# bastienjossen/DDL25Spring

Measured on AMD Instinct MI355X. Metric: FedAvg rounds/sec + local samples/sec, ResNet-18 CIFAR-10-shape, 8 clients, higher is better.
Workload: dtype fp32; 1 GPU; model=resnet18-cifar10, global_batch=800, parallelism=fedavg-8clients-dp1, clients=8, local_batch=100, local_epochs=1, samples_per_client=6250, client_slots_per_gpu=8, hip_graphs=True, fp32_conv_math=auto

## Files before the change

### csrc/include/conv_f32_core.h

```cpp
#pragma once
#include "ddl_common.h"

struct ConvF32Args {
  const float* x;
  const float* w;
  const float* dy;
  float* out;
  float* stats;
  const float* bias;
  const float* residual;
  const float* mask;
  const float* in_scale;
  const float* in_shift;
  const float* bn_x;
  const float* bn_mean;
  const float* bn_rstd;
  const float* mask_scale;
  const float* mask_shift;
  float* partial;
  long long partial_cap;
  long long x_gs, w_gs, dy_gs, out_gs, bias_gs, res_gs;
  int G, N, H, W, C, K, R, S, P, Q, stride, pad;
  int relu, accumulate, split_k, res_sub, in_relu;
  int slots;
  float gscale;
  const void* wsplit;
  long long ws_gs;
  const float* dyb_x;
  const float* dyb_coef;
  float* dyb_out;
  int* tickets;
  long long tickets_cap;
};

enum { F_FWD = 0, F_DGRAD = 1, F_WGRAD = 2 };

struct FDiv {
  uint32_t m;
  int s;
};
__host__ __device__ inline FDiv mk_fdiv(uint32_t d) {
  FDiv f;
  if (d <= 1) { f.m = 0; f.s = 0; return f; }
  int l = 0;
  while ((1u << l) < d) ++l;
  f.m = (uint32_t)((((1ull << 32) * ((1ull << l) - d)) / d) + 1);
  f.s = l;
  return f;
}
__device__ __forceinline__ int fdv(int x, FDiv f) {
  if (f.s == 0) return x;
  const uint32_t t = __umulhi((uint32_t)x, f.m);
  return (int)((t + (((uint32_t)x - t) >> 1)) >> (f.s - 1));
}

struct FGeo {
  int Pd, Qd, Kr, nph, phase, split, nsplit, g, p0, q0, tq;
  int pa, pb, Hs, Ws, r0, s0, Rn, Sn;
};

template <int MODE, int BP, int BQ>
__device__ __forceinline__ FGeo fgeo(const ConvF32Args& a, int bx, int by, int g, int gy) {
  FGeo o;
  o.nph = (MODE == F_DGRAD && a.stride == 2) ? 4 : 1;
  o.phase = by % o.nph;
  o.split = by / o.nph;
  o.nsplit = gy / o.nph;
  o.g = g;
  o.pa = o.pb = o.r0 = o.s0 = 0;
  o.Hs = a.H; o.Ws = a.W; o.Rn = a.R; o.Sn = a.S;
  if (MODE == F_FWD) {
    o.Pd = a.K; o.Qd = a.N * a.P * a.Q; o.Kr = a.R * a.S * a.C;
  } else if (MODE == F_DGRAD) {
    o.Pd = a.C;
    if (o.nph == 4) {
      o.pa = o.phase >> 1; o.pb = o.phase & 1;
      o.Hs = (a.H - o.pa + 1) >> 1; o.Ws = (a.W - o.pb + 1) >> 1;
      o.r0 = (o.pa + a.pad) & 1; o.s0 = (o.pb + a.pad) & 1;
      o.Rn = (a.R - o.r0 + 1) >> 1; o.Sn = (a.S - o.s0 + 1) >> 1;
    }
    o.Qd = a.N * o.Hs * o.Ws;
    o.Kr = o.Rn * o.Sn * a.K;
  } else {
    o.Pd = a.K; o.Qd = a.R * a.S * a.C; o.Kr = a.N * a.P * a.Q;
  }
// ... 224 lines not shown
    float* st = a.stats + ((long long)g * a.slots + slot) * 2 * Pd + o.p0 + tid;
    st[0] = t0;
    st[Pd] = t1;
  }
}

template <int MODE, int BP>
__device__ __forceinline__ void fzero_slot(const ConvF32Args& a, const FGeo& o) {
  if (MODE == F_WGRAD || !a.stats || (MODE == F_DGRAD && !a.bn_x)) return;
  const int tid = threadIdx.x;
  if (tid < BP && o.p0 + tid < o.Pd) {
    const int slot = o.phase * (a.slots / o.nph) + o.tq;
    float* st = a.stats + ((long long)o.g * a.slots + slot) * 2 * o.Pd + o.p0 + tid;
    st[0] = 0.f;
    st[o.Pd] = 0.f;
  }
}

template <int MODE, int BP, int BQ>
__global__ __launch_bounds__(256) void convf32_splitk_epilogue(ConvF32Args a) {
  constexpr int WP = BP / 2, WQ = BQ / 2, TP = WP / 16, TQ = WQ / 16;
  __shared__ float red[2 * BP * 2];
  const int tid = threadIdx.x, lane = tid & 63, wid = tid >> 6, wp = wid >> 1, wq = wid & 1;
  const int nph = (MODE == F_DGRAD && a.stride == 2) ? 4 : 1;
  const FGeo o = fgeo<MODE, BP, BQ>(a, blockIdx.x, blockIdx.y, blockIdx.z, nph * a.split_k);
  if (o.q0 >= o.Qd || o.p0 >= o.Pd) {
    fzero_slot<MODE, BP>(a, o);
    return;
  }
  const long long qmax = (long long)a.slots / nph * BQ;
  const long long slice = (long long)a.G * nph * qmax * o.Pd;
  const float* base = a.partial + ((long long)o.g * nph + o.phase) * qmax * o.Pd;
  f4v acc[TP][TQ];
  bool ok[TP][TQ];
  const float* src[TP][TQ];
#pragma unroll
  for (int ti = 0; ti < TP; ++ti)
#pragma unroll
    for (int tj = 0; tj < TQ; ++tj) {
      const int q = o.q0 + wq * WQ + tj * 16 + (lane & 15);
      const int p = o.p0 + wp * WP + ti * 16 + 4 * (lane >> 4);
      ok[ti][tj] = q < o.Qd && p < o.Pd;
      src[ti][tj] = base + (ok[ti][tj] ? (long long)q * o.Pd + p : 0);
      acc[ti][tj] = (f4v){0.f, 0.f, 0.f, 0.f};
    }
  for (int k = 0; k < a.split_k; ++k) {
    f4v v[TP][TQ];
#pragma unroll
    for (int ti = 0; ti < TP; ++ti)
#pragma unroll
      for (int tj = 0; tj < TQ; ++tj)
        v[ti][tj] = ok[ti][tj] ? *(const f4v*)(src[ti][tj] + k * slice) : (f4v){0.f, 0.f, 0.f, 0.f};
#pragma unroll
    for (int ti = 0; ti < TP; ++ti)
#pragma unroll
      for (int tj = 0; tj < TQ; ++tj) acc[ti][tj] += v[ti][tj];
  }
  fepi<MODE, BP, BQ, Lay16<BP, BQ>>(a, o, acc, red);
}


__device__ __forceinline__ void split3(float4 v, s4v& h, s4v& m, s4v& l) {
  const float x[4] = {v.x, v.y, v.z, v.w};
#pragma unroll
  for (int i = 0; i < 4; ++i) {
    const uint32_t u = __float_as_uint(x[i]);
    const float r1 = x[i] - __uint_as_float(u & 0xFFFF0000u);
    const uint32_t um = __float_as_uint(r1);
    const float r2 = r1 - __uint_as_float(um & 0xFFFF0000u);
    h[i] = (short)(u >> 16);
    m[i] = (short)(um >> 16);
    l[i] = (short)(__float_as_uint(r2) >> 16);
  }
}
__device__ __forceinline__ void split1(float x, uint16_t& h, uint16_t& m, uint16_t& l) {
  const uint32_t u = __float_as_uint(x);
  const float r1 = x - __uint_as_float(u & 0xFFFF0000u);
  const uint32_t um = __float_as_uint(r1);
  const float r2 = r1 - __uint_as_float(um & 0xFFFF0000u);
  h = (uint16_t)(u >> 16);
  m = (uint16_t)(um >> 16);
  l = (uint16_t)(__float_as_uint(r2) >> 16);
}
__device__ __forceinline__ s8v cat44(s4v a, s4v b) {
  return __builtin_shufflevector(a, b, 0, 1, 2, 3, 4, 5, 6, 7);
}
```

### csrc/kernels/conv_f32.hip

```cpp
#include "conv_f32_core.h"
#include <cstdlib>

#ifndef F32_PREFETCH
#define F32_PREFETCH 2
#endif

constexpr int FBK = 16;

__device__ __forceinline__ int fswz(int row) { return (row >> 2) & 2; }
__device__ __forceinline__ int lds_off(int row, int ch) { return row * 16 + ((ch ^ fswz(row)) << 2); }

__device__ __forceinline__ int x6_off(int row, int ch, int half) {
  const int f = row & 2;
  const int g = (row ^ (row >> 2)) & 1;
  return row * 32 + 8 * (ch ^ f) + 4 * (half ^ g);
}

template <int MODE, int BP, int BQ, int X6>
__global__ __launch_bounds__(256, (X6 && BP * BQ <= 64 * 128) ? 3 : 2) void convf32_kernel(ConvF32Args a) {
  constexpr int WP = BP / 2, WQ = BQ / 2, TP = WP / 16, TQ = WQ / 16;
  constexpr int RW = X6 ? 32 : 16;
  constexpr int SP = BP * RW, SQ = BQ * RW;
  constexpr int UPK = BP / 64, UQK = BQ / 64;
  constexpr int KUP = BP / 64, KUQ = BQ / 64;
  __shared__ float4 smem4[(2 * (SP + SQ)) / 4];
  float* smem = (float*)smem4;
  __shared__ float xform[2 * 512];

  const int tid = threadIdx.x, lane = tid & 63, wid = tid >> 6, wp = wid >> 1, wq = wid & 1;
  const int gx = gridDim.x, gy = gridDim.y, gz = gridDim.z;
  const int lin = blockIdx.x + gx * (blockIdx.y + gy * blockIdx.z);
  const int u = xcd_remap(lin, gx * gy * gz);
  const int bx = u % gx, by = (u / gx) % gy, g = u / (gx * gy);
  const FGeo o = fgeo<MODE, BP, BQ>(a, bx, by, g, gy);
  const bool split_store = a.split_k > 1;
  if (o.q0 >= o.Qd || o.p0 >= o.Pd) {
    if (!split_store || (a.tickets && o.split == 0)) fzero_slot<MODE, BP>(a, o);
    return;
  }
  const int nk = (o.Kr + FBK - 1) / FBK;
  const int per = (nk + o.nsplit - 1) / o.nsplit;
  const int kt0 = o.split * per, kt1 = min(nk, kt0 + per);

  const int H = a.H, W = a.W, C = a.C, K = a.K, S = a.S, P = a.P, Q = a.Q, st = a.stride, pd = a.pad;
  const float* X = a.x + (long long)g * a.x_gs;
  const float* Wt = a.w + (long long)g * a.w_gs;
  const float* DY = a.dy + (long long)g * a.dy_gs;
  const bool xf = (MODE != F_DGRAD) && a.in_scale != nullptr;
  if (xf) {
    for (int i = tid; i < C; i += 256) {
      xform[i] = a.in_scale[(long long)g * C + i];
      xform[512 + i] = a.in_shift[(long long)g * C + i];
    }
  }
  const bool xrelu = a.in_relu != 0;

  int pk_row[UPK], pk_ch[UPK];
  int pm_rg = 0, pm_kp = 0;
  if constexpr (MODE == F_FWD) {
#pragma unroll
    for (int i = 0; i < UPK; ++i) {
      const int uu = tid + 256 * i;
      pk_row[i] = uu >> 2;
      pk_ch[i] = uu & 3;
    }
  } else {
    pm_kp = tid % (16 / KUP);
    pm_rg = tid / (16 / KUP);
  }
  int qk_row[UQK], qk_ch[UQK], qk_n[UQK], qk_hb[UQK], qk_wb[UQK];
  int qm_rg = 0, qm_kp = 0, qm_r = 0, qm_s = 0, qm_c = 0;
  bool qm_ok = false;
  float qm_sc[4] = {1.f, 1.f, 1.f, 1.f}, qm_sh[4] = {0.f, 0.f, 0.f, 0.f};
  if constexpr (MODE != F_WGRAD) {
    const FDiv dpq = mk_fdiv((uint32_t)(MODE == F_FWD ? P * Q : o.Hs * o.Ws));
    const FDiv dq = mk_fdiv((uint32_t)(MODE == F_FWD ? Q : o.Ws));
    const int PQ = MODE == F_FWD ? P * Q : o.Hs * o.Ws, QQ = MODE == F_FWD ? Q : o.Ws;
#pragma unroll
    for (int i = 0; i < UQK; ++i) {
      const int uu = tid + 256 * i;
      qk_row[i] = uu >> 2;
      qk_ch[i] = uu & 3;
      const int q = o.q0 + qk_row[i];
      if (q < o.Qd) {
        const int n = fdv(q, dpq), rem = q - n * PQ;
        const int y = fdv(rem, dq), xq = rem - y * QQ;
        qk_n[i] = n;
        if (MODE == F_FWD) {
          qk_hb[i] = y * st - pd;
          qk_wb[i] = xq * st - pd;
        } else {
          qk_hb[i] = (o.nph == 4 ? 2 * y + o.pa : y) + pd;
          qk_wb[i] = (o.nph == 4 ? 2 * xq + o.pb : xq) + pd;
        }
      } else {
        qk_n[i] = -1;
        qk_hb[i] = qk_wb[i] = 0;
      }
    }
  } else {
    qm_kp = tid % (16 / KUQ);
    qm_rg = tid / (16 / KUQ);
    const int q = o.q0 + 4 * qm_rg;
    qm_ok = q < o.Qd;
    if (qm_ok) {
      const int tap = q / C;
      qm_c = q - tap * C;
      qm_r = tap / S;
      qm_s = tap - qm_r * S;
    }
  }
  if (xf) __syncthreads();
  if constexpr (MODE == F_WGRAD) {
    if (xf && qm_ok) {
#pragma unroll
      for (int v = 0; v < 4; ++v) { qm_sc[v] = xform[qm_c + v]; qm_sh[v] = xform[512 + qm_c + v]; }
    }
  }
  const FDiv dpix = mk_fdiv((uint32_t)(P * Q)), dpq1 = mk_fdiv((uint32_t)Q);

  constexpr unsigned OOB = 0xFFFFFFF0u;
  const __amdgpu_buffer_rsrc_t rX = __builtin_amdgcn_make_buffer_rsrc(
      (void*)X, 0, (int)((long long)a.N * H * W * C * 4), 0x00020000);
  const __amdgpu_buffer_rsrc_t rW = __builtin_amdgcn_make_buffer_rsrc(
      (void*)Wt, 0, (int)((long long)K * a.R * S * C * 4), 0x00020000);
  const __amdgpu_buffer_rsrc_t rD = __builtin_amdgcn_make_buffer_rsrc(
      (void*)DY, 0, (int)((long long)a.N * P * Q * K * 4), 0x00020000);
  auto bload = [&](const __amdgpu_buffer_rsrc_t& rs, unsigned off) -> float4 {
    const auto v = __builtin_amdgcn_raw_buffer_load_b128(rs, off, 0, 0);
    return __builtin_bit_cast(float4, v);
  };
  constexpr int PF = F32_PREFETCH;
  float4 rpA[2], rqA[2], rpB[2], rqB[2], rpC[2], rqC[2];
  bool qvA[2] = {false, false}, qvB[2] = {false, false}, qvC[2] = {false, false};
  auto load_step = [&](int kt, float4 (&rp)[2], float4 (&rq)[2], bool (&qv)[2]) {
    const int kk0 = kt * FBK;
    if constexpr (MODE == F_FWD) {
#pragma unroll
      for (int i = 0; i < UPK; ++i) {
        const int p = o.p0 + pk_row[i];
        rp[i] = bload(rW, p < o.Pd ? (unsigned)(p * o.Kr + kk0 + 4 * pk_ch[i]) * 4u : OOB);
      }
    } else if constexpr (MODE == F_DGRAD) {
      const int tap = kk0 / K, k0 = kk0 - tap * K;
      const int ir = tap / o.Sn, is = tap - ir * o.Sn;
      const int r = o.r0 + (st == 2 ? 2 : 1) * ir, s = o.s0 + (st == 2 ? 2 : 1) * is;
      const int c = o.p0 + 4 * pm_rg;
#pragma unroll
      for (int j = 0; j < KUP; ++j) {
        const int k = k0 + pm_kp * KUP + j;
        rp[j] = bload(rW, c < C ? (unsigned)(((k * a.R + r) * S + s) * C + c) * 4u : OOB);
      }
    } else {
      const int kch = o.p0 + 4 * pm_rg;
#pragma unroll
      for (int j = 0; j < KUP; ++j) {
        const int pix = kk0 + pm_kp * KUP + j;
        rp[j] = bload(rD, (pix < o.Kr && kch < K) ? (unsigned)(pix * K + kch) * 4u : OOB);
      }
    }
    if constexpr (MODE == F_FWD) {
      const int tap = kk0 / C, c0 = kk0 - tap * C;
      const int r = tap / S, s = tap - r * S;
#pragma unroll
      for (int i = 0; i < UQK; ++i) {
        const int h = qk_hb[i] + r, w = qk_wb[i] + s;
        const bool ok = qk_n[i] >= 0 && (unsigned)h < (unsigned)H && (unsigned)w < (unsigned)W;
        qv[i] = ok;
        rq[i] = bload(rX, ok ? (unsigned)(((qk_n[i] * H + h) * W + w) * C + c0 + 4 * qk_ch[i]) * 4u : OOB);
      }
    } else if constexpr (MODE == F_DGRAD) {
      const int tap = kk0 / K, k0 = kk0 - tap * K;
      const int ir = tap / o.Sn, is = tap - ir * o.Sn;
      const int r = o.r0 + (st == 2 ? 2 : 1) * ir, s = o.s0 + (st == 2 ? 2 : 1) * is;
#pragma unroll
      for (int i = 0; i < UQK; ++i) {
        int ho = qk_hb[i] - r, wo = qk_wb[i] - s;
        bool hit = true;
        if (st == 2) {
          ho >>= 1;
          wo >>= 1;
        } else if (st > 2) {
          hit = ho >= 0 && wo >= 0 && ho % st == 0 && wo % st == 0;
          ho /= st;
          wo /= st;
        }
        const bool ok = hit && qk_n[i] >= 0 && (unsigned)ho < (unsigned)P && (unsigned)wo < (unsigned)Q;
        rq[i] = bload(rD, ok ? (unsigned)(((qk_n[i] * P + ho) * Q + wo) * K + k0 + 4 * qk_ch[i]) * 4u : OOB);
      }
    } else {
#pragma unroll
      for (int j = 0; j < KUQ; ++j) {
        const int pix = kk0 + qm_kp * KUQ + j;
        const int n = fdv(pix, dpix), rem = pix - n * P * Q;
        const int ho = fdv(rem, dpq1), wo = rem - ho * Q;
        const int h = ho * st - pd + qm_r, w = wo * st - pd + qm_s;
        const bool ok = qm_ok && pix < o.Kr && (unsigned)h < (unsigned)H && (unsigned)w < (unsigned)W;
        qv[j] = ok;
        rq[j] = bload(rX, ok ? (unsigned)(((n * H + h) * W + w) * C + qm_c) * 4u : OOB);
      }
    }
  };
  auto xform4 = [&](float4 v, const float* sc, const float* sh) {
    v.x = v.x * sc[0] + sh[0];
    v.y = v.y * sc[1] + sh[1];
    v.z = v.z * sc[2] + sh[2];
    v.w = v.w * sc[3] + sh[3];
    if (xrelu) { v.x = fmaxf(v.x, 0.f); v.y = fmaxf(v.y, 0.f); v.z = fmaxf(v.z, 0.f); v.w = fmaxf(v.w, 0.f); }
    return v;
  };
  auto store_mn = [&](float* img, int rg, int kp, int KU, const float4* v) {
#pragma unroll
    for (int j4 = 0; j4 < 4; ++j4) {
      const int row = 4 * rg + j4;
      const int kk = kp * KU;
      float* d = img + row * 16 + (((kk >> 2) ^ fswz(row)) << 2) + (kk & 3);
      const float e0 = j4 == 0 ? v[0].x : j4 == 1 ? v[0].y : j4 == 2 ? v[0].z : v[0].w;
      if (KU == 2) {
        const float e1 = j4 == 0 ? v[1].x : j4 == 1 ? v[1].y : j4 == 2 ? v[1].z : v[1].w;
        *(float2*)d = make_float2(e0, e1);
      } else {
        *d = e0;
      }
    }
  };
  auto store_k6 = [&](float* img, int row, int ch, float4 v) {
    s4v h, m, l;
    split3(v, h, m, l);
    *(s8v*)(img + x6_off(row, ch, 0)) = cat44(h, m);
    *(s8v*)(img + x6_off(row, ch, 1)) = cat44(l, h);
  };
  auto store_mn6 = [&](float* img, int rg, int kp, int KU, const float4* v) {
#pragma unroll
    for (int j4 = 0; j4 < 4; ++j4) {
      const int row = 4 * rg + j4;
      const int kk = kp * KU, ch = kk >> 2, pos = kk & 3;
      uint16_t* h0 = (uint16_t*)(img + x6_off(row, ch, 0)) + pos;
      uint16_t* h1 = (uint16_t*)(img + x6_off(row, ch, 1)) + pos;
      const float e0 = j4 == 0 ? v[0].x : j4 == 1 ? v[0].y : j4 == 2 ? v[0].z : v[0].w;
      uint16_t ah, am, al;
      split1(e0, ah, am, al);
      if (KU == 2) {
        const float e1 = j4 == 0 ? v[1].x : j4 == 1 ? v[1].y : j4 == 2 ? v[1].z : v[1].w;
        uint16_t bh, bm, bl;
        split1(e1, bh, bm, bl);
        *(uint32_t*)h0 = (uint32_t)ah | ((uint32_t)bh << 16);
        *(uint32_t*)(h0 + 4) = (uint32_t)am | ((uint32_t)bm << 16);
        *(uint32_t*)h1 = (uint32_t)al | ((uint32_t)bl << 16);
        *(uint32_t*)(h1 + 4) = (uint32_t)ah | ((uint32_t)bh << 16);
      } else {
        h0[0] = ah;
        h0[4] = am;
        h1[0] = al;
        h1[4] = ah;
      }
    }
  };
  auto store_step = [&](int buf, int kt, float4 (&rp)[2], float4 (&rq)[2], const bool (&qv)[2]) {
    float* Ps = smem + buf * (SP + SQ);
    float* Qs = Ps + SP;
    if constexpr (MODE == F_FWD) {
#pragma unroll
      for (int i = 0; i < UPK; ++i) {
        if constexpr (X6) store_k6(Ps, pk_row[i], pk_ch[i], rp[i]);
        else *(float4*)(Ps + lds_off(pk_row[i], pk_ch[i])) = rp[i];
      }
    } else {
      if constexpr (X6) store_mn6(Ps, pm_rg, pm_kp, KUP, rp);
      else store_mn(Ps, pm_rg, pm_kp, KUP, rp);
    }
    if constexpr (MODE == F_FWD) {
      if (xf) {
        const int kk0 = kt * FBK, c0 = kk0 - (kk0 / C) * C;
#pragma unroll
        for (int i = 0; i < UQK; ++i) {
          const int c = c0 + 4 * qk_ch[i];
          if (qv[i]) rq[i] = xform4(rq[i], xform + c, xform + 512 + c);
        }
      }
    } else if constexpr (MODE == F_WGRAD) {
      if (xf) {
#pragma unroll
        for (int j = 0; j < KUQ; ++j)
          if (qv[j]) rq[j] = xform4(rq[j], qm_sc, qm_sh);
      }
    }
    if constexpr (MODE != F_WGRAD) {
#pragma unroll
      for (int i = 0; i < UQK; ++i) {
        if constexpr (X6) store_k6(Qs, qk_row[i], qk_ch[i], rq[i]);
        else *(float4*)(Qs + lds_off(qk_row[i], qk_ch[i])) = rq[i];
      }
    } else {
      if constexpr (X6) store_mn6(Qs, qm_rg, qm_kp, KUQ, rq);
      else store_mn(Qs, qm_rg, qm_kp, KUQ, rq);
    }
  };

  f4v acc[TP][TQ];
#pragma unroll
  for (int i = 0; i < TP; ++i)
#pragma unroll
    for (int j = 0; j < TQ; ++j) acc[i][j] = (f4v){0.f, 0.f, 0.f, 0.f};

  auto step = [&](int kt, float4 (&cp)[2], float4 (&cq)[2], bool (&cv)[2], float4 (&np)[2],
                  float4 (&nq)[2], bool (&nv)[2]) {
    const int cur = (kt - kt0) & 1;
    if (kt + PF < kt1) load_step(kt + PF, np, nq, nv);
    const float* Ps = smem + cur * (SP + SQ);
    const float* Qs = Ps + SP;
    if constexpr (X6) {
      s8v a0[TP], a1[TP], b0[TQ], b1[TQ];
#pragma unroll
      for (int ti = 0; ti < TP; ++ti) {
        const int R = wp * WP + ti * 16 + (lane & 15);
        a0[ti] = *(const s8v*)(Ps + x6_off(R, lane >> 4, 0));
        a1[ti] = *(const s8v*)(Ps + x6_off(R, lane >> 4, 1));
      }
#pragma unroll
      for (int tj = 0; tj < TQ; ++tj) {
        const int R = wq * WQ + tj * 16 + (lane & 15);
        b0[tj] = *(const s8v*)(Qs + x6_off(R, lane >> 4, 0));
        b1[tj] = *(const s8v*)(Qs + x6_off(R, lane >> 4, 1));
      }
#pragma unroll
      for (int ti = 0; ti < TP; ++ti)
#pragma unroll
        for (int tj = 0; tj < TQ; ++tj) {
          f4v c = __builtin_amdgcn_mfma_f32_16x16x32_bf16(a1[ti], b0[tj], (f4v){0.f, 0.f, 0.f, 0.f}, 0, 0, 0);
          c = __builtin_amdgcn_mfma_f32_16x16x32_bf16(a0[ti], b1[tj], c, 0, 0, 0);
          c = __builtin_amdgcn_mfma_f32_16x16x32_bf16(a0[ti], b0[tj], c, 0, 0, 0);
#pragma unroll
          for (int v = 0; v < 4; ++v) acc[ti][tj][v] = acc[ti][tj][v] + c[v];
        }
    } else {
      float4 af[TP], bfr[TQ];
#pragma unroll
      for (int ti = 0; ti < TP; ++ti)
        af[ti] = *(const float4*)(Ps + lds_off(wp * WP + ti * 16 + (lane & 15), lane >> 4));
#pragma unroll
      for (int tj = 0; tj < TQ; ++tj)
        bfr[tj] = *(const float4*)(Qs + lds_off(wq * WQ + tj * 16 + (lane & 15), lane >> 4));
#pragma unroll
      for (int s4 = 0; s4 < 4; ++s4)
#pragma unroll
        for (int ti = 0; ti < TP; ++ti)
#pragma unroll
          for (int tj = 0; tj < TQ; ++tj) {
            const float av = s4 == 0 ? af[ti].x : s4 == 1 ? af[ti].y : s4 == 2 ? af[ti].z : af[ti].w;
            const float bv = s4 == 0 ? bfr[tj].x : s4 == 1 ? bfr[tj].y : s4 == 2 ? bfr[tj].z : bfr[tj].w;
            acc[ti][tj] = __builtin_amdgcn_mfma_f32_16x16x4f32(av, bv, acc[ti][tj], 0, 0, 0);
          }
    }
    if (kt + 1 < kt1) store_step(cur ^ 1, kt + 1, cp, cq, cv);
    __syncthreads();
  };
  if (kt0 < kt1) {
    load_step(kt0, rpA, rqA, qvA);
    if (kt0 + 1 < kt1) load_step(kt0 + 1, rpB, rqB, qvB);
    if constexpr (PF == 3) {
      if (kt0 + 2 < kt1) load_step(kt0 + 2, rpC, rqC, qvC);
    }
    store_step(0, kt0, rpA, rqA, qvA);
    __syncthreads();
    if constexpr (PF == 3) {
      for (int kt = kt0; kt < kt1; kt += 3) {
        step(kt, rpB, rqB, qvB, rpA, rqA, qvA);
        if (kt + 1 < kt1) step(kt + 1, rpC, rqC, qvC, rpB, rqB, qvB);
        if (kt + 2 < kt1) step(kt + 2, rpA, rqA, qvA, rpC, rqC, qvC);
      }
    } else {
      for (int kt = kt0; kt < kt1; kt += 2) {
        step(kt, rpB, rqB, qvB, rpA, rqA, qvA);
        if (kt + 1 < kt1) step(kt + 1, rpA, rqA, qvA, rpB, rqB, qvB);
      }
    }
  }

  if (split_store) {
#pragma unroll
    for (int ti = 0; ti < TP; ++ti)
#pragma unroll
      for (int tj = 0; tj < TQ; ++tj) {
        const int q = o.q0 + wq * WQ + tj * 16 + (lane & 15);
        const int p = o.p0 + wp * WP + ti * 16 + 4 * (lane >> 4);
        if (q >= o.Qd || p >= o.Pd) continue;
        if constexpr (MODE == F_WGRAD) {
          float* d = a.partial + ((long long)o.split * a.G + g) * o.Pd * o.Qd;
#pragma unroll
          for (int v = 0; v < 4; ++v)
            if (p + v < o.Pd) d[(long long)(p + v) * o.Qd + q] = acc[ti][tj][v];
        } else {
          const long long qmax = (long long)a.slots / o.nph * BQ;
          float* d = a.partial + (((long long)o.split * a.G + g) * o.nph + o.phase) * qmax * o.Pd;
          *(float4*)(d + (long long)q * o.Pd + p) = make_float4(acc[ti][tj][0], acc[ti][tj][1],
                                                                acc[ti][tj][2], acc[ti][tj][3]);
        }
      }
    if (a.tickets) {
      __threadfence();
      __syncthreads();
      int* const last = (int*)smem;
      int* const ticket = a.tickets + ((long long)g * o.nph + o.phase) * gx + bx;
      if (tid == 0) *last = atomicAdd(ticket, 1) == o.nsplit - 1;
      __syncthreads();
      if (!*last) return;
      __threadfence();
      if constexpr (MODE != F_WGRAD) {
        const long long qmax = (long long)a.slots / o.nph * BQ;
        const long long slice = (long long)a.G * o.nph * qmax * o.Pd;
        const float* base = a.partial + ((long long)g * o.nph + o.phase) * qmax * o.Pd;
#pragma unroll
        for (int ti = 0; ti < TP; ++ti)
#pragma unroll
          for (int tj = 0; tj < TQ; ++tj) {
            const int q = o.q0 + wq * WQ + tj * 16 + (lane & 15);
            const int p = o.p0 + wp * WP + ti * 16 + 4 * (lane >> 4);
            f4v sm = (f4v){0.f, 0.f, 0.f, 0.f};
            if (q < o.Qd && p < o.Pd) {
              const float* src = base + (long long)q * o.Pd + p;
              for (int k = 0; k < o.nsplit; ++k) {
                const float4 v = *(const float4*)(src + k * slice);
                sm[0] += v.x; sm[1] += v.y; sm[2] += v.z; sm[3] += v.w;
              }
            }
            acc[ti][tj] = sm;
          }
        __syncthreads();
        if (tid == 0) *ticket = 0;
        fepi<MODE, BP, BQ, Lay16<BP, BQ>>(a, o, acc, smem);
        return;
      } else {
        const long long per = (long long)o.Pd * o.Qd;
        const float* src = a.partial + (long long)g * per;
        float* dst = a.out + (long long)g * a.out_gs;
        for (int e = tid; e < BP * (BQ / 4); e += 256) {
          const int p = o.p0 + e / (BQ / 4), q = o.q0 + 4 * (e % (BQ / 4));
          if (p >= o.Pd || q >= o.Qd) continue;
          const long long off = (long long)p * o.Qd + q;
          float4 sum = make_float4(0.f, 0.f, 0.f, 0.f);
          for (int k = 0; k < o.nsplit; ++k) {
            const float4 v = *(const float4*)(src + (long long)k * a.G * per + off);
            sum.x += v.x; sum.y += v.y; sum.z += v.z; sum.w += v.w;
          }
          float4 b = a.accumulate ? *(const float4*)(dst + off) : make_float4(0.f, 0.f, 0.f, 0.f);
          b.x += a.gscale * sum.x; b.y += a.gscale * sum.y; b.z += a.gscale * sum.z; b.w += a.gscale * sum.w;
          *(float4*)(dst + off) = b;
        }
        if (tid == 0) *ticket = 0;
      }
    }
    return;
  }
  fepi<MODE, BP, BQ, Lay16<BP, BQ>>(a, o, acc, smem);
}

template <int V>
__global__ __launch_bounds__(256) void convf32_wgrad_reduce(const float* __restrict__ part, float* out,
                                                            long long out_gs, int G, long long nv,
                                                            int splits, int accumulate, float gscale) {
  typedef float vec __attribute__((ext_vector_type(V)));
  const long long per = nv * V;
  GSTRIDE_LOOP(t, (long long)G * nv) {
    const long long g = t / nv, i = (t - g * nv) * V;
    vec s = (vec)(0.f);
    const float* src = part + g * per + i;
    const long long sstride = (long long)G * per;
    int k = 0;
    for (; k + 8 <= splits; k += 8) {
      vec v[8];
#pragma unroll
      for (int j = 0; j < 8; ++j) v[j] = *(const vec*)(src + (long long)(k + j) * sstride);
#pragma unroll
      for (int j = 0; j < 8; ++j) s += v[j];
    }
    for (; k < splits; ++k) s += *(const vec*)(src + (long long)k * sstride);
    float* d = out + g * out_gs + i;
    vec b = accumulate ? *(const vec*)d : (vec)(0.f);
    b += gscale * s;
    *(vec*)d = b;
  }
}

static void launch_wgrad_reduce(const float* part, float* out, long long out_gs, int G, long long n, int splits,
                                int accumulate, float gscale, hipStream_t s) {
  static const long long v4_min = [] {
    const char* e = getenv("DDL_WGRAD_REDUCE_V4_MIN");
    return e ? atoll(e) : 512LL * 256;
  }();
  if ((long long)G * (n / 4) >= v4_min)
    hipLaunchKernelGGL(convf32_wgrad_reduce<4>, dim3(grid_for((long long)G * (n / 4), 256)), dim3(256), 0, s, part,
                       out, out_gs, G, n / 4, splits, accumulate, gscale);
  else
    hipLaunchKernelGGL(convf32_wgrad_reduce<1>, dim3(grid_for((long long)G * n, 256)), dim3(256), 0, s, part, out,
                       out_gs, G, n, splits, accumulate, gscale);
}

DDL_API int ddl_convf32_wgrad_reduce(const float* part, float* out, long long out_gs, int G, long long n, int splits,
                                     int accumulate, float gscale, hipStream_t s) {
  if (n % 4) return (int)hipErrorInvalidValue;
  launch_wgrad_reduce(part, out, out_gs, G, n, splits, accumulate, gscale, s);
  return (int)hipGetLastError();
}

static void fdims(const ConvF32Args& a, int mode, long long& Pd, long long& Qd, long long& Qmax, long long& Kr,
                  int& nph) {
  nph = (mode == F_DGRAD && a.stride == 2) ? 4 : 1;
  if (mode == F_FWD) { Pd = a.K; Qd = Qmax = (long long)a.N * a.P * a.Q; Kr = (long long)a.R * a.S * a.C; }
  else if (mode == F_DGRAD) {
    Pd = a.C;
    const int Hs = nph == 4 ? (a.H + 1) >> 1 : a.H, Ws = nph == 4 ? (a.W + 1) >> 1 : a.W;
    Qd = Qmax = (long long)a.N * Hs * Ws;
    Kr = (long long)a.R * a.S * a.K;
  } else { Pd = a.K; Qd = Qmax = (long long)a.R * a.S * a.C; Kr = (long long)a.N * a.P * a.Q; }
}

DDL_API long long ddl_convf32_slots(const ConvF32Args* ap, int mode, int cfg) {
  long long Pd, Qd, Qmax, Kr;
  int nph;
  fdims(*ap, mode, Pd, Qd, Qmax, Kr, nph);
  const int bq = ((cfg >> 8) & 0xff) * 16;
  if (bq <= 0) return -1;
  return nph * ((Qmax + bq - 1) / bq);
}

DDL_API long long ddl_convf32_workspace(const ConvF32Args* ap, int mode, int cfg) {
  if (ap->split_k <= 1) return 0;
  long long Pd, Qd, Qmax, Kr;
  int nph;
  fdims(*ap, mode, Pd, Qd, Qmax, Kr, nph);
  const int bq = ((cfg >> 8) & 0xff) * 16;
  if (mode == F_WGRAD) return (long long)ap->split_k * ap->G * Pd * Qd;
  const long long qm = (Qmax + bq - 1) / bq * bq;
  return (long long)ap->split_k * ap->G * nph * qm * Pd;
}

template <int MODE, int BP, int BQ, int X6>
static int launch_tile(ConvF32Args a, hipStream_t s) {
  long long Pd, Qd, Qmax, Kr;
  int nph;
  fdims(a, MODE, Pd, Qd, Qmax, Kr, nph);
  const long long ntp = (Pd + BP - 1) / BP, ntq = (Qmax + BQ - 1) / BQ;
  a.slots = (int)(nph * ntq);
  const int split = a.split_k < 1 ? 1 : a.split_k;
  a.split_k = split;
  if (split > 1) {
    const long long need = MODE == F_WGRAD ? (long long)split * a.G * Pd * Qd
                                           : (long long)split * a.G * nph * ntq * BQ * Pd;
    if (!a.partial || need > a.partial_cap) return (int)hipErrorInvalidValue;
  }
  const dim3 grid((unsigned)(ntp * ntq), (unsigned)(nph * split), (unsigned)a.G);
  if (split == 1 || (long long)a.G * nph * ntp * ntq > a.tickets_cap) a.tickets = nullptr;
  hipLaunchKernelGGL((convf32_kernel<MODE, BP, BQ, X6>), grid, dim3(256), 0, s, a);
  hipError_t e = hipGetLastError();
  if (e != hipSuccess || split == 1 || a.tickets) return (int)e;
  if (MODE == F_WGRAD) {
    launch_wgrad_reduce((const float*)a.partial, a.out, a.out_gs, a.G, Pd * Qd, split, a.accumulate, a.gscale, s);
  } else {
    hipLaunchKernelGGL((convf32_splitk_epilogue<MODE, BP, BQ>), dim3((unsigned)(ntp * ntq), nph, a.G),
                       dim3(256), 0, s, a);
  }
  return (int)hipGetLastError();
}

template <int MODE, int X6>
static int launch_math(const ConvF32Args& a, int bp, int bq, hipStream_t s) {
  if (bp == 64 && bq == 64) return launch_tile<MODE, 64, 64, X6>(a, s);
  if (bp == 64 && bq == 128) return launch_tile<MODE, 64, 128, X6>(a, s);
  if (bp == 128 && bq == 64) return launch_tile<MODE, 128, 64, X6>(a, s);
  if (bp == 128 && bq == 128) return launch_tile<MODE, 128, 128, X6>(a, s);
  return (int)hipErrorInvalidValue;
}

template <int MODE>
static int launch_mode(const ConvF32Args& a, int cfg, hipStream_t s) {
  const int bp = (cfg & 0xff) * 16, bq = ((cfg >> 8) & 0xff) * 16;
  return (cfg >> 16) & 1 ? launch_math<MODE, 1>(a, bp, bq, s) : launch_math<MODE, 0>(a, bp, bq, s);
}

DDL_API int ddl_convf32(const ConvF32Args* ap, int mode, int cfg, hipStream_t s) {
  const ConvF32Args& a = *ap;
  if (a.G < 1 || a.N < 1 || a.C < 1 || a.K < 1 || a.stride < 1) return (int)hipErrorInvalidValue;
  if (a.C > 512 && a.in_scale) return (int)hipErrorInvalidValue;
  const long long lim = (1LL << 31) - 64;
  if ((long long)a.N * a.H * a.W * a.C * 4 > lim || (long long)a.K * a.R * a.S * a.C * 4 > lim ||
      (long long)a.N * a.P * a.Q * a.K * 4 > lim)
    return (int)hipErrorInvalidValue;
  if (mode == F_FWD) {
    if (a.C % 16 || a.K % 4) return (int)hipErrorInvalidValue;
    return launch_mode<F_FWD>(a, cfg, s);
  }
  if (mode == F_DGRAD) {
    if (a.K % 16 || a.C % 4) return (int)hipErrorInvalidValue;
    return launch_mode<F_DGRAD>(a, cfg, s);
  }
  if (mode == F_WGRAD) {
    if (a.C % 4 || a.K % 4) return (int)hipErrorInvalidValue;
    if (!a.accumulate && a.gscale != 1.f) return (int)hipErrorInvalidValue;
    return launch_mode<F_WGRAD>(a, cfg, s);
  }
  return (int)hipErrorInvalidValue;
}

DDL_API int ddl_convf32_args_size() { return (int)sizeof(ConvF32Args); }
```

### ddl25spring_amd/ops/functional_f32.py

```python
from __future__ import annotations

import ctypes
import math
import os

import torch

from . import _lib
from . import workspace as ws
from ._lib import check, ptr, stream

F_FWD, F_DGRAD, F_WGRAD = 0, 1, 2
WS_CAP = 1 << 26
_WS: dict = {}
TARGET_WG = int(os.environ.get("DDL_F32_TARGET_WG", "640"))


def is_f32(t) -> bool:
    return t is not None and t.is_cuda and t.dtype == torch.float32


class SlotStats:
    __slots__ = ("t", "rows")

    def __init__(self):
        self.t = None
        self.rows = 0


def workspace(device, role: str = "main") -> torch.Tensor:
    key = f"{device}:{role}"
    b = _WS.get(key)
    if b is None:
        if torch.cuda.is_current_stream_capturing():
            raise RuntimeError("fp32 split-K workspace first requested inside a graph capture: run one eager "
                               "step (or functional_f32.ensure_workspace) before capturing")
        ensure_workspace(device)
        b = _WS[key]
    return b


def ensure_workspace(device) -> None:
    for role in ("main", "side"):
        key = f"{device}:{role}"
        if key not in _WS:
            _WS[key] = torch.empty(WS_CAP, dtype=torch.float32, device=device)
            _WS[key + ":tickets"] = torch.zeros(TICKETS_CAP, dtype=torch.int32, device=device)
    if torch.device(device).type == "cuda" and _dev_key(device) not in _TICKETS:
        _TICKETS[_dev_key(device)] = torch.zeros(TICKETS_N, dtype=torch.int32, device=device)


TICKETS_CAP = 1 << 18
WG_FOLD = [os.environ.get("DDL_F32_WG_FOLD", "0") == "1"]


def _dims(mode, g):
    if mode == F_FWD:
        return g.K, g.N * g.P * g.Q, g.R * g.S * g.C, 1
    if mode == F_DGRAD:
        if g.stride == 2:
            hs, wsz = (g.H + 1) // 2, (g.W + 1) // 2
            rn, sn = (g.R + 1) // 2, (g.S + 1) // 2
            return g.C, g.N * hs * wsz, rn * sn * g.K, 4
        return g.C, g.N * g.H * g.W, g.R * g.S * g.K, 1
    return g.K, g.R * g.S * g.C, g.N * g.P * g.Q, 1


def cfg_of(bp: int, bq: int) -> int:
    return (bp // 16) | ((bq // 16) << 8)


MATHS = ("mfma32", "x6", "auto")
_MATH = [os.environ.get("DDL_F32_MATH", "auto")]
if _MATH[0] not in MATHS:
    raise ValueError(f"DDL_F32_MATH={_MATH[0]!r}: expected one of {MATHS}")


def math() -> str:
    return _MATH[0]


def set_math(name: str) -> None:
    if name not in MATHS:
        raise ValueError(f"fp32 conv math {name!r}: expected one of {MATHS}")
    if name != _MATH[0]:
        _MATH[0] = name
        _PLANS.clear()


X6_BIT = 1 << 16
HALO_BIT = 1 << 17
_HALO = [os.environ.get("DDL_F32_HALO", "1") != "0"]
HALO_HPMAX = 288


def set_halo(on: bool) -> None:
    if bool(on) != _HALO[0]:
        _HALO[0] = bool(on)
        _PLANS.clear()


HALO_MIN_W = int(os.environ.get("DDL_F32_HALO_MIN_W", "4"))
HALO_PADW = [os.environ.get("DDL_F32_HALO_PADW", "1") != "0"]


def halo_ok(mode: int, g, auto: bool = False) -> bool:
    if mode not in (F_FWD, F_DGRAD) or g.stride != 1 or g.R != g.S or g.R not in (1, 3) or g.pad != (g.R - 1) // 2:
        return False
    if g.P != g.H or g.Q != g.W:
        return False
    OH, OWr = g.P, g.Q
    if OWr < 4 or OWr > 128:
        return False
    if auto and OWr < HALO_MIN_W:
        return False
    OW = 1 << (OWr - 1).bit_length()
    if OW != OWr and (not HALO_PADW[0] or (auto and g.R == 1)):
        return False
    TR = 128 // OW
    if TR <= OH:
        if OH % TR:
            return False
        SR = TR
    else:
        if TR % OH:
            return False
        SR = OH
    HP = (TR // SR) * (SR + g.R - 1) * (OW + g.S - 1)
    SC, Pd = (g.C, g.K) if mode == F_FWD else (g.K, g.C)
    if not (HP <= HALO_HPMAX and SC % 16 == 0 and Pd % 4 == 0):
        return False
    return _x6h_native_ok(mode, g)


_X6H_OK: dict = {}


def _x6h_native_ok(mode: int, g) -> bool:
    key = (mode, g)
    r = _X6H_OK.get(key)
    if r is None:
        try:
            lib = _lib.kernels()
        except Exception:
            return True
        a = _args(g)
        r = bool(lib.ddl_x6h_ok(ctypes.byref(a), mode, cfg_of(64, 128)))
        _X6H_OK[key] = r
    return r


HALO_TINY, HALO_SMALL, HALO_LARGE = 26624, 32768, 45056


def halo_layout(mode: int, geom, bp: int = 64):
    out = (ctypes.c_int * 5)()
    a = _args(geom)
    if _lib.kernels().ddl_x6h_layout(ctypes.byref(a), mode, cfg_of(bp, 128), out) != 0:
        return None
    return dict(zip(("ROWB", "SEGB", "HBYTES", "HP", "tier"), out))


def halo_residency(mode: int, bp: int, rs: int, tier: int, padw: bool = False) -> int:
    return int(_lib.kernels().ddl_x6h_residency(mode, bp, rs, tier, int(padw)))


_FLAT_ENV = os.environ.get("DDL_F32_FLAT1X1", "fd")
FLAT1X1 = [_FLAT_ENV != "0", "fdw" if _FLAT_ENV == "1" else _FLAT_ENV]


def _launch_geom(geom, mode: str = "f"):
    if not FLAT1X1[0] or mode not in FLAT1X1[1] or geom.R != 1 or geom.S != 1 or geom.stride != 1 or geom.pad != 0:
        return geom
    if geom.W & (geom.W - 1) == 0 and geom.W <= 128:
        return geom
# ... 80 lines not shown
    key = (mode, geom)
    p = _PLANS.get(key)
    if p is not None:
        return p
    if _RECORD_PATH:
        _RECORDED.add(key)
    p = _OVERRIDE.get(key)
    if p is None and _HALO[0] and _MATH[0] != "mfma32" and halo_ok(mode, geom, auto=True):
        p = _halo_plan(mode, geom)
    if p is None:
        p = _tuned(mode, geom)
    if p is None:
        Pd, Qd, Kr, nph = _dims(mode, geom)
        bp = 128 if Pd > 64 else 64
        bq = 128 if Qd > 64 else 64
        tiles = -(-Pd // bp) * -(-Qd // bq) * nph * geom.G
        nk = -(-Kr // 16)
        split = 1
        while tiles * split < TARGET_WG and nk >= split * 2 * 8 and split < 64:
            split *= 2
        p = (cfg_of(bp, bq) | X6_BIT, split)
    _PLANS[key] = p
    return p


def _halo_plan(mode: int, geom) -> tuple[int, int]:
    _tuned(mode, geom)
    if TARGET_WG != 1:
        p = _TUNED.get(f"x6h:{_MODE_NAMES[mode]}:{geom.G},{geom.N},{geom.H},{geom.W},{geom.C},{geom.K},"
                       f"{geom.R},{geom.S},{geom.stride},{geom.pad}")
        if p is not None:
            return cfg_of(int(p[0]), int(p[1])) | X6_BIT | HALO_BIT, int(p[2])
    Pd, Qd, _, _ = _dims(mode, geom)
    SC = geom.C if mode == F_FWD else geom.K
    bp = 128 if Pd > 64 and geom.Q > 4 else 64
    tiles = -(-Pd // bp) * -(-Qd // 128) * geom.G
    nch = SC // 16
    split = 1
    padded = geom.Q & (geom.Q - 1) != 0
    while not padded and tiles * split < TARGET_WG and nch >= split * 2 * 4 and split < 32:
        split *= 2
    return cfg_of(bp, 128) | X6_BIT | HALO_BIT, split


def _args(geom, **kw) -> _lib.ConvF32Args:
    a = _lib.ConvF32Args()
    a.gscale = 1.0
    for k, v in kw.items():
        setattr(a, k, v)
    a.G, a.N, a.H, a.W, a.C, a.K = geom.G, geom.N, geom.H, geom.W, geom.C, geom.K
    a.R, a.S, a.P, a.Q, a.stride, a.pad = geom.R, geom.S, geom.P, geom.Q, geom.stride, geom.pad
    return a


def _gs(t) -> int:
    return 0 if t is None else t.stride(0)


def _launch(a, mode: int, geom, device, split_k: int = 0, ws_role: str = "main") -> None:
    lib = _lib.kernels()
    cfg, split = plan(mode, geom)
    if split_k:
        split = split_k
    a.split_k = split
    cfg = _cfg(cfg)
    if cfg & HALO_BIT and not halo_ok(mode, geom):
        cfg &= ~HALO_BIT
    if split > 1:
        need = lib.ddl_convf32_workspace(ctypes.byref(a), mode, cfg)
        buf = workspace(device, ws_role)
        if need > buf.numel():
            a.split_k = split = 1
        else:
            a.partial, a.partial_cap = buf.data_ptr(), buf.numel()
            if WG_FOLD[0] and not (cfg & HALO_BIT):
                t = _WS[f"{device}:{ws_role}:tickets"]
                a.tickets, a.tickets_cap = t.data_ptr(), t.numel()
    name = ("conv_fwd", "conv_dgrad", "conv_wgrad")[mode] + "_f32"
    if cfg & HALO_BIT:
        ws_buf = split_weights(a, mode, geom, device)
        a.wsplit, a.ws_gs = ws_buf.data_ptr(), ws_buf.stride(0)
        check(lib.ddl_x6h(ctypes.byref(a), mode, cfg & ~HALO_BIT, stream()), name + "_halo")
        return
    check(lib.ddl_convf32(ctypes.byref(a), mode, cfg, stream()), name)


def split_weights(a, mode: int, geom, device) -> torch.Tensor:
    T = geom.R * geom.S
    layout = 0 if mode == F_FWD else 1
    scope = _PRESPLIT[0]
    if scope is not None:
        key = (int(a.w), layout, geom.G, geom.K, T, geom.C, int(a.w_gs))
        buf = scope.lookup(key)
        if buf is not None:
            return buf
    out = torch.empty(geom.G, geom.K * T * geom.C * 6, dtype=torch.uint8, device=device)
    check(_lib.kernels().ddl_x6_split_weights(a.w, out.data_ptr(), geom.G, geom.K, T, geom.C, 0 if mode == F_FWD else 1,
                                              a.w_gs, out.stride(0), 0, stream()), "x6_split_weights")
    return out


class _SplitDesc(ctypes.Structure):
    _fields_ = [("w", ctypes.c_void_p), ("out", ctypes.c_void_p), ("w_gs", ctypes.c_longlong),
                ("o_gs", ctypes.c_longlong), ("G", ctypes.c_int), ("K", ctypes.c_int), ("T", ctypes.c_int),
                ("C", ctypes.c_int), ("layout", ctypes.c_int), ("blk0", ctypes.c_int), ("nblk", ctypes.c_int),
                ("pad_", ctypes.c_int)]


_PRESPLIT: list = [None]
PRESPLIT = [os.environ.get("DDL_F32_PRESPLIT", "1") != "0"]
PRESPLIT_SIDE = [os.environ.get("DDL_F32_PRESPLIT_SIDE", "0") == "1"]
PRESPLIT_HEAD_FRAC = float(os.environ.get("DDL_F32_PRESPLIT_HEAD", "0.05"))
_SPLIT_STREAMS: dict = {}


class PresplitScope:

    def __init__(self):
        self.keys: list = []
        self._seen: set = set()
        self.bufs: dict = {}
        self.tables: list = []
        self.tail: set = set()
        self._pending = None
        self.state = "record"
        self._prev = None

    def lookup(self, key):
        if self.state == "ready":
            if self._pending is not None and key in self.tail:
                torch.cuda.current_stream().wait_event(self._pending)
                self._pending = None
            return self.bufs.get(key)
        if key not in self._seen:
            self._seen.add(key)
            self.keys.append(key)
        return None

    def __enter__(self):
        self._prev = _PRESPLIT[0]
        if not PRESPLIT[0]:
            return self
        if self.state == "ready":
            lib = _lib.kernels()
            desc, n, nb = self.tables[0]
            check(lib.ddl_x6_split_weights_multi(ptr(desc), n, nb, stream()), "x6_split_weights_multi")
            if len(self.tables) > 1:
                cur = torch.cuda.current_stream()
                side = _SPLIT_STREAMS.get(cur.device)
                if side is None:
                    side = _SPLIT_STREAMS[cur.device] = torch.cuda.Stream(device=cur.device)
                side.wait_stream(cur)
                desc, n, nb = self.tables[1]
                with torch.cuda.stream(side):
                    check(lib.ddl_x6_split_weights_multi(ptr(desc), n, nb, stream()), "x6_split_weights_multi")
                    ev = torch.cuda.Event()
                    ev.record(side)
                self._pending = ev
        _PRESPLIT[0] = self
        return self

    def __exit__(self, *exc):
        _PRESPLIT[0] = self._prev
        if self._pending is not None:
            torch.cuda.current_stream().wait_event(self._pending)
            self._pending = None
# ... 453 lines not shown
```

Before: 42660 samples/s.

## Add incremental-address wgrad staging path with paired bf16x3 split stores

Adds a new wgrad staging variant for the X6 (bf16x3 split) fp32 conv kernel, enabled by default. Per-step pixel index divisions are replaced by an incremental walker that advances buffer offsets with carry logic. The input transform is specialized at compile time for no transform, scale/shift, or scale/shift+relu. When the unroll factor is 2, two elements are split and packed per LDS store using byte perms. The cost is more template instantiations and registers, and loads now run past the end of the K loop with masking.

```diff
diff --git a/csrc/include/conv_f32_core.h b/csrc/include/conv_f32_core.h
--- a/csrc/include/conv_f32_core.h
+++ b/csrc/include/conv_f32_core.h
@@ -1,6 +1,59 @@
 #pragma once
+#ifdef CONVF32_WALK_ONLY
+#include <stdint.h>
+#define F32_HD inline
+#else
 #include "ddl_common.h"
-
+#define F32_HD __host__ __device__ inline
+#endif
+
+struct XWalk {
+  int dw, dh;
+  int qs, ps;
+  int st;
+  uint32_t doff, wcar, hcar;
+};
+struct XPix {
+  int h, w;
+  uint32_t off;
+};
+F32_HD XWalk xwalk_make(int H, int W, int C, int P, int Q, int st, int adv) {
+  const int PQ = P * Q, dn = adv / PQ, r = adv - dn * PQ, dh = r / Q, dw = r - dh * Q;
+  const uint32_t c4 = 4u * (uint32_t)C;
+  XWalk k;
+  k.dw = dw * st;
+  k.dh = dh * st;
+  k.qs = Q * st;
+  k.ps = P * st;
+  k.st = st;
+  k.doff = c4 * ((uint32_t)dn * (uint32_t)H * (uint32_t)W + (uint32_t)(dh * st) * (uint32_t)W + (uint32_t)(dw * st));
+  k.wcar = c4 * ((uint32_t)st * (uint32_t)W - (uint32_t)(Q * st));
+  k.hcar = c4 * ((uint32_t)H * (uint32_t)W - (uint32_t)(P * st) * (uint32_t)W);
+  return k;
+}
+F32_HD XPix xwalk_init(int n, int ho, int wo, int r, int s, int c, int H, int W, int C, int st, int pd) {
+  XPix p;
+  p.h = ho * st - pd + r;
+  p.w = wo * st - pd + s;
+  p.off = ((((uint32_t)n * (uint32_t)H + (uint32_t)p.h) * (uint32_t)W + (uint32_t)p.w) * (uint32_t)C + (uint32_t)c) * 4u;
+  return p;
+}
+F32_HD void xwalk_advance(XPix& p, const XWalk& k, int hlim, int wlim) {
+  p.w += k.dw;
+  p.off += k.doff;
+  const bool cw = p.w >= wlim;
+  p.w -= cw ? k.qs : 0;
+  p.h += k.dh + (cw ? k.st : 0);
+  p.off += cw ? k.wcar : 0u;
+  const bool ch = p.h >= hlim;
+  p.h -= ch ? k.ps : 0;
+  p.off += ch ? k.hcar : 0u;
+}
+F32_HD bool xwalk_inside(const XPix& p, int H, int W) {
+  return ((uint32_t)p.h < (uint32_t)H) & ((uint32_t)p.w < (uint32_t)W);
+}
+
+#ifndef CONVF32_WALK_ONLY
 struct ConvF32Args {
   const float* x;
   const float* w;
@@ -391,6 +444,19 @@
   m = (uint16_t)(um >> 16);
   l = (uint16_t)(__float_as_uint(r2) >> 16);
 }
+__device__ __forceinline__ void split2(float a, float b, uint32_t& h, uint32_t& m, uint32_t& l) {
+  constexpr uint32_t HI2 = 0x07060302u;
+  const uint32_t ua = __float_as_uint(a), ub = __float_as_uint(b);
+  const float a1 = a - __uint_as_float(ua & 0xFFFF0000u);
+  const float b1 = b - __uint_as_float(ub & 0xFFFF0000u);
+  const uint32_t uam = __float_as_uint(a1), ubm = __float_as_uint(b1);
+  const float a2 = a1 - __uint_as_float(uam & 0xFFFF0000u);
+  const float b2 = b1 - __uint_as_float(ubm & 0xFFFF0000u);
+  h = __builtin_amdgcn_perm(ub, ua, HI2);
+  m = __builtin_amdgcn_perm(ubm, uam, HI2);
+  l = __builtin_amdgcn_perm(__float_as_uint(b2), __float_as_uint(a2), HI2);
+}
 __device__ __forceinline__ s8v cat44(s4v a, s4v b) {
   return __builtin_shufflevector(a, b, 0, 1, 2, 3, 4, 5, 6, 7);
 }
+#endif
diff --git a/csrc/kernels/conv_f32.hip b/csrc/kernels/conv_f32.hip
--- a/csrc/kernels/conv_f32.hip
+++ b/csrc/kernels/conv_f32.hip
@@ -16,8 +16,12 @@
   return row * 32 + 8 * (ch ^ f) + 4 * (half ^ g);
 }
 
-template <int MODE, int BP, int BQ, int X6>
+template <int N>
+struct IC { static constexpr int value = N; };
+
+template <int MODE, int BP, int BQ, int X6, int STG = 0>
 __global__ __launch_bounds__(256, (X6 && BP * BQ <= 64 * 128) ? 3 : 2) void convf32_kernel(ConvF32Args a) {
+  constexpr bool NS = STG == 1 && MODE == F_WGRAD && X6 == 1;
   constexpr int WP = BP / 2, WQ = BQ / 2, TP = WP / 16, TQ = WQ / 16;
   constexpr int RW = X6 ? 32 : 16;
   constexpr int SP = BP * RW, SQ = BQ * RW;
@@ -118,6 +122,27 @@
     }
   }
   const FDiv dpix = mk_fdiv((uint32_t)(P * Q)), dpq1 = mk_fdiv((uint32_t)Q);
+  XWalk xw;
+  XPix xpx[KUQ];
+  int x_hlim = 0, x_wlim = 0, x_rem = 0, d_rem = 0;
+  uint32_t d_off = 0;
+  if constexpr (NS) {
+    xw = xwalk_make(H, W, C, P, Q, st, FBK);
+    x_hlim = P * st - pd + qm_r;
+    x_wlim = Q * st - pd + qm_s;
+    const int pixq = kt0 * FBK + qm_kp * KUQ;
+    x_rem = qm_ok ? o.Kr - pixq : 0;
+#pragma unroll
+    for (int j = 0; j < KUQ; ++j) {
+      const int pix = pixq + j;
+      const int n = fdv(pix, dpix), rem = pix - n * P * Q;
+      const int ho = fdv(rem, dpq1), wo = rem - ho * Q;
+      xpx[j] = xwalk_init(n, ho, wo, qm_r, qm_s, qm_c, H, W, C, st, pd);
+    }
+    const int pixp = kt0 * FBK + pm_kp * KUP, kch = o.p0 + 4 * pm_rg;
+    d_rem = kch < K ? o.Kr - pixp : 0;
+    d_off = ((uint32_t)pixp * (uint32_t)K + (uint32_t)kch) * 4u;
+  }
 
   constexpr unsigned OOB = 0xFFFFFFF0u;
   const __amdgpu_buffer_rsrc_t rX = __builtin_amdgcn_make_buffer_rsrc(
@@ -151,6 +176,12 @@
         const int k = k0 + pm_kp * KUP + j;
         rp[j] = bload(rW, c < C ? (unsigned)(((k * a.R + r) * S + s) * C + c) * 4u : OOB);
       }
+    } else if constexpr (NS) {
+#pragma unroll
+      for (int j = 0; j < KUP; ++j)
+        rp[j] = bload(rD, d_rem > j ? d_off + (uint32_t)(j * K) * 4u : OOB);
+      d_off += (uint32_t)(FBK * K) * 4u;
+      d_rem -= FBK;
     } else {
       const int kch = o.p0 + 4 * pm_rg;
 #pragma unroll
@@ -188,6 +219,15 @@
         const bool ok = hit && qk_n[i] >= 0 && (unsigned)ho < (unsigned)P && (unsigned)wo < (unsigned)Q;
         rq[i] = bload(rD, ok ? (unsigned)(((qk_n[i] * P + ho) * Q + wo) * K + k0 + 4 * qk_ch[i]) * 4u : OOB);
       }
+    } else if constexpr (NS) {
+#pragma unroll
+      for (int j = 0; j < KUQ; ++j) {
+        const bool ok = (x_rem > j) & xwalk_inside(xpx[j], H, W);
+        qv[j] = ok;
+        rq[j] = bload(rX, ok ? xpx[j].off : OOB);
+        xwalk_advance(xpx[j], xw, x_hlim, x_wlim);
+      }
+      x_rem -= FBK;
     } else {
 #pragma unroll
       for (int j = 0; j < KUQ; ++j) {
@@ -207,6 +247,21 @@
     v.z = v.z * sc[2] + sh[2];
     v.w = v.w * sc[3] + sh[3];
     if (xrelu) { v.x = fmaxf(v.x, 0.f); v.y = fmaxf(v.y, 0.f); v.z = fmaxf(v.z, 0.f); v.w = fmaxf(v.w, 0.f); }
+    return v;
+  };
+  auto xform4s = [&](float4 v, bool real, auto relu) {
+    float4 t;
+    t.x = v.x * qm_sc[0] + qm_sh[0];
+    t.y = v.y * qm_sc[1] + qm_sh[1];
+    t.z = v.z * qm_sc[2] + qm_sh[2];
+    t.w = v.w * qm_sc[3] + qm_sh[3];
+    if constexpr (decltype(relu)::value) {
+      t.x = fmaxf(t.x, 0.f); t.y = fmaxf(t.y, 0.f); t.z = fmaxf(t.z, 0.f); t.w = fmaxf(t.w, 0.f);
+    }
+    v.x = real ? t.x : v.x;
+    v.y = real ? t.y : v.y;
+    v.z = real ? t.z : v.z;
+    v.w = real ? t.w : v.w;
     return v;
   };
   auto store_mn = [&](float* img, int rg, int kp, int KU, const float4* v) {
@@ -256,7 +311,25 @@
       }
     }
   };
-  auto store_step = [&](int buf, int kt, float4 (&rp)[2], float4 (&rq)[2], const bool (&qv)[2]) {
+  auto store_mn6p = [&](float* img, int rg, int kp, const float4* v) {
+#pragma unroll
+    for (int j4 = 0; j4 < 4; ++j4) {
+      const int row = 4 * rg + j4;
+      const int kk = kp * 2, ch = kk >> 2, pos = (kk & 3) >> 1;
+      uint32_t* h0 = (uint32_t*)(img + x6_off(row, ch, 0)) + pos;
+      uint32_t* h1 = (uint32_t*)(img + x6_off(row, ch, 1)) + pos;
+      const float e0 = j4 == 0 ? v[0].x : j4 == 1 ? v[0].y : j4 == 2 ? v[0].z : v[0].w;
+      const float e1 = j4 == 0 ? v[1].x : j4 == 1 ? v[1].y : j4 == 2 ? v[1].z : v[1].w;
+      uint32_t ph, pm, pl;
+      split2(e0, e1, ph, pm, pl);
+      h0[0] = ph;
+      h0[2] = pm;
+      h1[0] = pl;
+      h1[2] = ph;
+    }
+  };
+  auto store_step = [&](int buf, int kt, float4 (&rp)[2], float4 (&rq)[2], const bool (&qv)[2], auto xm) {
+    constexpr int XM = decltype(xm)::value;
     float* Ps = smem + buf * (SP + SQ);
     float* Qs = Ps + SP;
     if constexpr (MODE == F_FWD) {
@@ -266,7 +339,8 @@
         else *(float4*)(Ps + lds_off(pk_row[i], pk_ch[i])) = rp[i];
       }
     } else {
-      if constexpr (X6) store_mn6(Ps, pm_rg, pm_kp, KUP, rp);
+      if constexpr (NS && KUP == 2) store_mn6p(Ps, pm_rg, pm_kp, rp);
+      else if constexpr (X6) store_mn6(Ps, pm_rg, pm_kp, KUP, rp);
       else store_mn(Ps, pm_rg, pm_kp, KUP, rp);
     }
     if constexpr (MODE == F_FWD) {
@@ -278,6 +352,11 @@
           if (qv[i]) rq[i] = xform4(rq[i], xform + c, xform + 512 + c);
         }
       }
+    } else if constexpr (NS) {
+      if constexpr (XM > 0) {
+#pragma unroll
+        for (int j = 0; j < KUQ; ++j) rq[j] = xform4s(rq[j], qv[j], IC<XM == 2>{});
+      }
     } else if constexpr (MODE == F_WGRAD) {
       if (xf) {
 #pragma unroll
@@ -292,7 +371,8 @@
         else *(float4*)(Qs + lds_off(qk_row[i], qk_ch[i])) = rq[i];
       }
     } else {
-      if constexpr (X6) store_mn6(Qs, qm_rg, qm_kp, KUQ, rq);
+      if constexpr (NS && KUQ == 2) store_mn6p(Qs, qm_rg, qm_kp, rq);
+      else if constexpr (X6) store_mn6(Qs, qm_rg, qm_kp, KUQ, rq);
       else store_mn(Qs, qm_rg, qm_kp, KUQ, rq);
     }
   };
@@ -304,9 +384,9 @@
     for (int j = 0; j < TQ; ++j) acc[i][j] = (f4v){0.f, 0.f, 0.f, 0.f};
 
   auto step = [&](int kt, float4 (&cp)[2], float4 (&cq)[2], bool (&cv)[2], float4 (&np)[2],
-                  float4 (&nq)[2], bool (&nv)[2]) {
+                  float4 (&nq)[2], bool (&nv)[2], auto xm) {
     const int cur = (kt - kt0) & 1;
-    if (kt + PF < kt1) load_step(kt + PF, np, nq, nv);
+    if (NS || kt + PF < kt1) load_step(kt + PF, np, nq, nv);
     const float* Ps = smem + cur * (SP + SQ);
     const float* Qs = Ps + SP;
     if constexpr (X6) {
@@ -352,30 +432,39 @@
             acc[ti][tj] = __builtin_amdgcn_mfma_f32_16x16x4f32(av, bv, acc[ti][tj], 0, 0, 0);
           }
     }
-    if (kt + 1 < kt1) store_step(cur ^ 1, kt + 1, cp, cq, cv);
+    if (NS || kt + 1 < kt1) store_step(cur ^ 1, kt + 1, cp, cq, cv, xm);
     __syncthreads();
   };
-  if (kt0 < kt1) {
-    load_step(kt0, rpA, rqA, qvA);
-    if (kt0 + 1 < kt1) load_step(kt0 + 1, rpB, rqB, qvB);
-    if constexpr (PF == 3) {
-      if (kt0 + 2 < kt1) load_step(kt0 + 2, rpC, rqC, qvC);
-    }
-    store_step(0, kt0, rpA, rqA, qvA);
-    __syncthreads();
-    if constexpr (PF == 3) {
-      for (int kt = kt0; kt < kt1; kt += 3) {
-        step(kt, rpB, rqB, qvB, rpA, rqA, qvA);
-        if (kt + 1 < kt1) step(kt + 1, rpC, rqC, qvC, rpB, rqB, qvB);
-        if (kt + 2 < kt1) step(kt + 2, rpA, rqA, qvA, rpC, rqC, qvC);
-      }
-    } else {
-      for (int kt = kt0; kt < kt1; kt += 2) {
-        step(kt, rpB, rqB, qvB, rpA, rqA, qvA);
-        if (kt + 1 < kt1) step(kt + 1, rpA, rqA, qvA, rpB, rqB, qvB);
-      }
-    }
-  }
+#define F32_MAIN_LOOP(xm)                                                       \
+  if (kt0 < kt1) {                                                              \
+    load_step(kt0, rpA, rqA, qvA);                                              \
+    if (kt0 + 1 < kt1) load_step(kt0 + 1, rpB, rqB, qvB);                       \
+    if constexpr (PF == 3) {                                                    \
+      if (kt0 + 2 < kt1) load_step(kt0 + 2, rpC, rqC, qvC);                     \
+    }                                                                           \
+    store_step(0, kt0, rpA, rqA, qvA, xm);                                      \
+    __syncthreads();                                                            \
+    if constexpr (PF == 3) {                                                    \
+      for (int kt = kt0; kt < kt1; kt += 3) {                                   \
+        step(kt, rpB, rqB, qvB, rpA, rqA, qvA, xm);                             \
+        if (kt + 1 < kt1) step(kt + 1, rpC, rqC, qvC, rpB, rqB, qvB, xm);       \
+        if (kt + 2 < kt1) step(kt + 2, rpA, rqA, qvA, rpC, rqC, qvC, xm);       \
+      }                                                                         \
+    } else {                                                                    \
+      for (int kt = kt0; kt < kt1; kt += 2) {                                   \
+        step(kt, rpB, rqB, qvB, rpA, rqA, qvA, xm);                             \
+        if (kt + 1 < kt1) step(kt + 1, rpA, rqA, qvA, rpB, rqB, qvB, xm);       \
+      }                                                                         \
+    }                                                                           \
+  }
+  if constexpr (NS) {
+    if (!xf) { F32_MAIN_LOOP(IC<0>{}) }
+    else if (!xrelu) { F32_MAIN_LOOP(IC<1>{}) }
+    else { F32_MAIN_LOOP(IC<2>{}) }
+  } else {
+    F32_MAIN_LOOP(IC<-1>{})
+  }
+#undef F32_MAIN_LOOP
 
   if (split_store) {
 #pragma unroll
@@ -535,7 +624,7 @@
   return (long long)ap->split_k * ap->G * nph * qm * Pd;
 }
 
-template <int MODE, int BP, int BQ, int X6>
+template <int MODE, int BP, int BQ, int X6, int STG = 0>
 static int launch_tile(ConvF32Args a, hipStream_t s) {
   long long Pd, Qd, Qmax, Kr;
   int nph;
@@ -551,7 +640,7 @@
   }
   const dim3 grid((unsigned)(ntp * ntq), (unsigned)(nph * split), (unsigned)a.G);
   if (split == 1 || (long long)a.G * nph * ntp * ntq > a.tickets_cap) a.tickets = nullptr;
-  hipLaunchKernelGGL((convf32_kernel<MODE, BP, BQ, X6>), grid, dim3(256), 0, s, a);
+  hipLaunchKernelGGL((convf32_kernel<MODE, BP, BQ, X6, STG>), grid, dim3(256), 0, s, a);
   hipError_t e = hipGetLastError();
   if (e != hipSuccess || split == 1 || a.tickets) return (int)e;
   if (MODE == F_WGRAD) {
@@ -563,19 +652,23 @@
   return (int)hipGetLastError();
 }
 
-template <int MODE, int X6>
+template <int MODE, int X6, int STG>
 static int launch_math(const ConvF32Args& a, int bp, int bq, hipStream_t s) {
-  if (bp == 64 && bq == 64) return launch_tile<MODE, 64, 64, X6>(a, s);
-  if (bp == 64 && bq == 128) return launch_tile<MODE, 64, 128, X6>(a, s);
-  if (bp == 128 && bq == 64) return launch_tile<MODE, 128, 64, X6>(a, s);
-  if (bp == 128 && bq == 128) return launch_tile<MODE, 128, 128, X6>(a, s);
+  if (bp == 64 && bq == 64) return launch_tile<MODE, 64, 64, X6, STG>(a, s);
+  if (bp == 64 && bq == 128) return launch_tile<MODE, 64, 128, X6, STG>(a, s);
+  if (bp == 128 && bq == 64) return launch_tile<MODE, 128, 64, X6, STG>(a, s);
+  if (bp == 128 && bq == 128) return launch_tile<MODE, 128, 128, X6, STG>(a, s);
   return (int)hipErrorInvalidValue;
 }
 
 template <int MODE>
 static int launch_mode(const ConvF32Args& a, int cfg, hipStream_t s) {
   const int bp = (cfg & 0xff) * 16, bq = ((cfg >> 8) & 0xff) * 16;
-  return (cfg >> 16) & 1 ? launch_math<MODE, 1>(a, bp, bq, s) : launch_math<MODE, 0>(a, bp, bq, s);
+  if (!((cfg >> 16) & 1)) return launch_math<MODE, 0, 0>(a, bp, bq, s);
+  if constexpr (MODE == F_WGRAD) {
+    if (!((cfg >> 18) & 1)) return launch_math<MODE, 1, 1>(a, bp, bq, s);
+  }
+  return launch_math<MODE, 1, 0>(a, bp, bq, s);
 }
 
 DDL_API int ddl_convf32(const ConvF32Args* ap, int mode, int cfg, hipStream_t s) {
diff --git a/ddl25spring_amd/ops/functional_f32.py b/ddl25spring_amd/ops/functional_f32.py
--- a/ddl25spring_amd/ops/functional_f32.py
+++ b/ddl25spring_amd/ops/functional_f32.py
@@ -91,6 +91,11 @@
 X6_BIT = 1 << 16
 HALO_BIT = 1 << 17
 _HALO = [os.environ.get("DDL_F32_HALO", "1") != "0"]
+STAGE_LEGACY_BIT = 1 << 18
+WGRAD_STAGE = os.environ.get("DDL_F32_WGRAD_STAGE", "new")
+if WGRAD_STAGE not in ("new", "legacy"):
+    raise ValueError(f"DDL_F32_WGRAD_STAGE={WGRAD_STAGE!r}: expected 'new' or 'legacy'")
+WGRAD_STAGE_LEGACY = [WGRAD_STAGE == "legacy"]
 HALO_HPMAX = 288
 
 
@@ -337,6 +342,8 @@
         a.wsplit, a.ws_gs = ws_buf.data_ptr(), ws_buf.stride(0)
         check(lib.ddl_x6h(ctypes.byref(a), mode, cfg & ~HALO_BIT, stream()), name + "_halo")
         return
+    if mode == F_WGRAD and WGRAD_STAGE_LEGACY[0]:
+        cfg |= STAGE_LEGACY_BIT
     check(lib.ddl_convf32(ctypes.byref(a), mode, cfg, stream()), name)
 
 
```

After: 42860 samples/s, median of 6. No clear change (+0.5%).
